# semihkacmaz/CoNFiLD

Hardware: AMD Instinct MI355X
Metric: generated fields/sec (256-step sample + CNF decode), Case4 latent, 1/2/4/8 GPU (higher is better)
Workload: dtype f32

## Files before the change

confild_amd/csrc/conv_x.hip:

```cpp
#include <algorithm>
#include <type_traits>

#include "unet_kernels.hpp"

namespace cfd {

typedef float f16v __attribute__((ext_vector_type(16)));
typedef float f2 __attribute__((ext_vector_type(2)));
typedef _Float16 h2 __attribute__((ext_vector_type(2)));
typedef unsigned u4 __attribute__((ext_vector_type(4)));

__device__ __forceinline__ int xswz(int row, int chunk) { return row * 64 + ((chunk ^ ((row >> 2) & 3)) << 4); }

__device__ __forceinline__ void split4_mix_x(const f4& x, uint2& hi, uint2& lo) {
    hi.x = __builtin_bit_cast(unsigned, __builtin_convertvector((f2){x[0], x[1]}, h2));
    hi.y = __builtin_bit_cast(unsigned, __builtin_convertvector((f2){x[2], x[3]}, h2));
    asm("v_fma_mixlo_f16 %0, %1, 1.0, -%2 op_sel_hi:[0,0,1]" : "=&v"(lo.x) : "v"(x[0]), "v"(hi.x));
    asm("v_fma_mixhi_f16 %0, %1, 1.0, -%2 op_sel:[0,0,1] op_sel_hi:[0,0,1]" : "+v"(lo.x) : "v"(x[1]), "v"(hi.x));
    asm("v_fma_mixlo_f16 %0, %1, 1.0, -%2 op_sel_hi:[0,0,1]" : "=&v"(lo.y) : "v"(x[2]), "v"(hi.y));
    asm("v_fma_mixhi_f16 %0, %1, 1.0, -%2 op_sel:[0,0,1] op_sel_hi:[0,0,1]" : "+v"(lo.y) : "v"(x[3]), "v"(hi.y));
}

__device__ __forceinline__ float phase_scale(const ConvArgs& a, int ph) {
    return ph == 0 ? a.ph_scale[0] : ph == 1 ? a.ph_scale[1] : ph == 2 ? a.ph_scale[2] : a.ph_scale[3];
}

template <int BM, int BN, int WGM, int WGN, int PF = 1, bool PH = false>
__global__ __launch_bounds__(64 * WGM * WGN, 1) void conv_x_kernel(ConvArgs a) {
    constexpr int NW = WGM * WGN, NT = 64 * NW;
    constexpr int WTM = BM / WGM, WTN = BN / WGN;
    constexpr int TM = WTM / 32, TN = WTN / 32;
    constexpr int RPP = NT / 8;
    constexpr int AIT = BM / RPP, BIT = BN / RPP;
    static_assert(TM >= 1 && TN >= 1 && AIT >= 1 && BIT >= 1, "tile");
    static_assert(BM % RPP == 0 && BN % RPP == 0, "staging");
    constexpr int ABYTES = BM * 64, BBYTES = BN * 64;
    constexpr int STAGE = 2 * ABYTES + 2 * BBYTES;
    __shared__ __attribute__((aligned(16))) char lds[2 * STAGE];

    CFD_STAMP(a.stamps, 2, a.seq, 0);
    const int tid = threadIdx.x, lane = tid & 63;
    const int wave = __builtin_amdgcn_readfirstlane(tid >> 6);
    const int wm = wave / WGN, wn = wave % WGN;

    int bx, by, bz;
    xcd_tile(a.xcd, bx, by, bz);
    const int ph = PH ? bx & 3 : 0, py = ph >> 1, px = ph & 1;
    if constexpr (PH) bx >>= 2;
    const int m0 = bx * BM, n0 = by * BN;
    const int HWo = a.Hout * a.Wout;
    const int HWm = PH ? a.Hin * a.Win : HWo, Wm = PH ? a.Win : a.Wout, Mm = PH ? a.M >> 2 : a.M;
    const int kq = tid & 7, rsub = tid >> 3;
    __shared__ int pixtab[(PH ? 4 : 9) * BM];

    const int srows = __builtin_amdgcn_readfirstlane(a.Hin * a.Win * (a.M / HWo));
// ... 176 lines not shown
    for (int i = 0; i < TM; ++i)
#pragma unroll
        for (int j = 0; j < TN; ++j) acc[i][j] *= PH ? phase_scale(a, ph) : a.acc_scale;
    const int n_base = n0 + wn * WTN + l32;
    const int m_base = m0 + wm * WTM + 4 * hsel;
    auto orow = [&](int mm, int& bb) __attribute__((always_inline)) {
        bb = mm / HWm;
        if constexpr (!PH) return mm;
        const int rem = mm - bb * HWm, y = rem / Wm, x = rem - y * Wm;
        return (bb * a.Hout + 2 * y + py) * a.Wout + 2 * x + px;
    };
    if (gridDim.z > 1) {
        float* part = a.part + (int64_t)bz * a.M * a.Cout;
#pragma unroll
        for (int i = 0; i < TM; ++i)
#pragma unroll
            for (int e = 0; e < 16; ++e) {
                const int mm = m_base + 32 * i + 8 * (e >> 2) + (e & 3);
                if (mm >= Mm) continue;
                int bb;
                const int m = orow(mm, bb);
#pragma unroll
                for (int j = 0; j < TN; ++j) {
                    const int n = n_base + 32 * j;
                    if (n < a.Cout) part[(int64_t)m * a.Cout + n] = acc[i][j][e];
                }
            }
#ifdef CFD_STAMPS
        __builtin_amdgcn_s_waitcnt(0);
#endif
        CFD_STAMP(a.stamps, 2, a.seq, 4);
        return;
    }
#pragma unroll
    for (int i = 0; i < TM; ++i)
#pragma unroll
        for (int e = 0; e < 16; ++e) {
            const int mm = m_base + 32 * i + 8 * (e >> 2) + (e & 3);
            if (mm >= Mm) continue;
            int bb;
            const int m = orow(mm, bb);
#pragma unroll
            for (int j = 0; j < TN; ++j) {
                const int n = n_base + 32 * j;
                if (n >= a.Cout) continue;
                float v = a.bias ? acc[i][j][e] + a.bias[n] : acc[i][j][e];
                if (a.emb) v = v + a.emb[(int64_t)bb * a.emb_stride + n];
                if (a.res) v = a.res[(int64_t)m * a.Cout + n] + v;
                a.out[(int64_t)m * a.Cout + n] = v;
            }
        }
}

template <int BM, int TW, bool BF = false, bool SB = false, int BN = 128, bool PH = false>
__global__ __launch_bounds__(BM * (BN / 64), 1) void conv_h_kernel(ConvArgs a) {
    static_assert(!SB || BF, "a bf16 source needs the bf16 kernel");
    static_assert(!PH || !BF, "the phase form is split-f16 only");
    constexpr unsigned SES = SB ? 2u : 4u;
    constexpr int WGN = BN / 64, WGM = BM / 64, NTG = 64 * WGM * WGN;
    static_assert(BN == 64 || BN == 128, "K1h: 64 or 128 output channels per workgroup");
    constexpr int PL = BF ? 1 : 2;
    constexpr int HW2 = TW < 32 ? (TW + 2 + 3) / 4 * 4 : TW + 2;
    constexpr int TR = BM / TW, NPX = (TR + 2) * HW2;
    auto hswz = [](int px, int hr, int chunk) __attribute__((always_inline)) {
        if constexpr (TW == 16) return px * 64 + ((chunk ^ (((px >> 2) + 3 * hr) & 3)) << 4);
        else return xswz(px, chunk);
    };
    constexpr int HPLANE = NPX * 64;
    constexpr int HIT = (NPX * 8 + NTG - 1) / NTG;
    constexpr int NTAP = PH ? 4 : 9;
    constexpr int TG = BF ? 3 : 1, SPR = NTAP / TG;
    constexpr int BPLANE = BN * 64, BSTAGE = PL * BPLANE * TG;
    constexpr int BIT = BN * 4 / NTG;
    constexpr int GBYTES = PL * HPLANE + 2 * BSTAGE;
    static_assert(BM % TW == 0 && BIT >= 1, "tile");
    __shared__ __attribute__((aligned(16))) char lds[GBYTES];

    CFD_STAMP(a.stamps, 3, a.seq, 0);
    const int tid = threadIdx.x, lane = tid & 63;
    const int wave = __builtin_amdgcn_readfirstlane(tid >> 6);
    const int wm = wave / WGN, wn = wave % WGN;
    const int gt = tid;
    char* const halo = lds;
    char* const ring = halo + PL * HPLANE;
    int bx, by, bz;
    xcd_tile(a.xcd, bx, by, bz);
    const int ph = PH ? bx & 3 : 0, py = ph >> 1, px = ph & 1;
    if constexpr (PH) bx >>= 2;
    const int n0 = by * BN;
    const int W = PH ? a.Win : a.Wout, Hh = PH ? a.Hin : a.Hout, HWo = Hh * W;
    const int tps = HWo / BM, tpr = W / TW;
    const int bimg = bx / tps, tl = bx - bimg * tps;
    const int y0 = (tl / tpr) * TR, x0 = (tl - (tl / tpr) * tpr) * TW;
    const int64_t mrow0 = PH ? ((int64_t)bimg * a.Hout + 2 * y0 + py) * a.Wout + 2 * x0 + px
                             : (int64_t)bimg * HWo + (int64_t)y0 * W + x0;
    CFD_DASSERT(mrow0 + (int64_t)(PH ? 2 : 1) * ((int64_t)(TR - 1) * a.Wout + TW - 1) < a.M && HWo % BM == 0 &&
                W % TW == 0);

    const int srows = __builtin_amdgcn_readfirstlane(a.Hin * a.Win * (a.M / (a.Hout * a.Wout)));
    const __amdgpu_buffer_rsrc_t rs1 = __builtin_amdgcn_make_buffer_rsrc((void*)a.src1, 0, srows * a.C1 * SES, 0x00020000);
    const __amdgpu_buffer_rsrc_t rs2 = __builtin_amdgcn_make_buffer_rsrc(
        (void*)(a.src2 ? (const void*)a.src2 : (const void*)a.src1), 0, a.src2 ? srows * a.C2 * SES : 0, 0x00020000);
    const int wbytes = a.Cout * NTAP * a.Ctot * 2;
    const char* const wh0 = PH ? (const char*)a.wph + (int64_t)ph * wbytes : (const char*)a.wbf;
    const char* const wl0 = PH ? (const char*)a.wpl + (int64_t)ph * wbytes : (const char*)a.wlo;
    const __amdgpu_buffer_rsrc_t rwh = __builtin_amdgcn_make_buffer_rsrc((void*)wh0, 0, wbytes, 0x00020000);
    const __amdgpu_buffer_rsrc_t rwl = __builtin_amdgcn_make_buffer_rsrc((void*)wl0, 0, wbytes, 0x00020000);

// ... 267 lines not shown
                const int64_t m = pix_of(p_base + 32 * i + 8 * (e >> 2) + (e & 3));
#pragma unroll
                for (int j = 0; j < 2; ++j) {
                    const int n = n_base + 32 * j;
                    if (n < a.Cout) part[(int64_t)m * a.Cout + n] = acc[i][j][e];
                }
            }
#ifdef CFD_STAMPS
        __builtin_amdgcn_s_waitcnt(0);
#endif
        CFD_STAMP(a.stamps, 3, a.seq, 4);
        return;
    }
#pragma unroll
    for (int i = 0; i < 2; ++i)
#pragma unroll
        for (int e = 0; e < 16; ++e) {
            const int64_t m = pix_of(p_base + 32 * i + 8 * (e >> 2) + (e & 3));
#pragma unroll
            for (int j = 0; j < 2; ++j) {
                const int n = n_base + 32 * j;
                if (n >= a.Cout) continue;
                float v = a.bias ? acc[i][j][e] + a.bias[n] : acc[i][j][e];
                if (a.emb) v = v + a.emb[(int64_t)bimg * a.emb_stride + n];
                if (a.res) v = a.res[(int64_t)m * a.Cout + n] + v;
                a.out[(int64_t)m * a.Cout + n] = v;
            }
        }
#ifdef CFD_STAMPS
    __builtin_amdgcn_s_waitcnt(0);
#endif
    CFD_STAMP(a.stamps, 3, a.seq, 4);
}

int conv_h_tw(const ConvArgs& a) {
    const bool geo = !a.tmode && a.ks == 3 && a.stride == 1 && a.pad == 1 && a.C1 % 32 == 0 && a.C2 % 32 == 0 &&
                     (a.up ? a.Hout == 2 * a.Hin && a.Wout == 2 * a.Win : a.Hout == a.Hin && a.Wout == a.Win) &&
                     a.M % (a.Hout * a.Wout) == 0;
    if (!geo) return 0;
    for (int tw = 64; tw >= 16; tw >>= 1)
        if (a.Wout % tw == 0 && a.Hout % (256 / tw) == 0) return tw;
    return 0;
}

int conv_hp_tw(const ConvArgs& a) {
    const bool geo = !a.tmode && a.up && a.ks == 3 && a.stride == 1 && a.pad == 1 && a.C1 % 32 == 0 &&
                     a.C2 % 32 == 0 && a.Hout == 2 * a.Hin && a.Wout == 2 * a.Win && a.M % (a.Hout * a.Wout) == 0;
    if (!geo) return 0;
    for (int tw = 64; tw >= 16; tw >>= 1)
        if (a.Win % tw == 0 && a.Hin % (256 / tw) == 0) return tw;
    return 0;
}

int launch_conv_x(const ConvArgs& a, int variant, int splits, hipStream_t st) {
    CFD_REQUIRE(a.wbf && !a.tmode, CFD_ESTATE, "conv_x: split-f16 or bf16 forward only");
    CFD_REQUIRE(a.Ctot % 32 == 0 && a.C1 % 4 == 0 && a.C2 % 4 == 0, CFD_ESHAPE, "conv_x needs channels % 32 == 0");
    CFD_REQUIRE(splits == 1 || a.part, CFD_ESTATE, "split-K needs a partial buffer");
    {
        const int64_t srows = (int64_t)a.Hin * a.Win * (a.M / (a.Hout * a.Wout));
        CFD_REQUIRE(srows < (1 << 24) && srows * std::max(a.C1, a.C2) * 4 < (1ll << 31) &&
                        (int64_t)a.Cout * a.K * 2 < (1ll << 31) && a.ks * a.ks <= 9,
                    CFD_ESHAPE, "conv_x: operands beyond 2 GiB");
    }
    auto grid = [&](int bm, int bn) __attribute__((always_inline)) {
        return dim3((unsigned)ceil_div(a.M, bm), (unsigned)ceil_div(a.Cout, bn), splits);
    };
    if (variant == 22) {
        const int tw = conv_h_tw(a);
        CFD_REQUIRE(tw > 0 && !a.wlo, CFD_ESHAPE, "conv_h bf16: 3x3 stride-1 with a 16/32/64-divisible width");
        const dim3 g = grid(256, 128);
        if (a.src_bf16) {
            if (tw == 64) hipLaunchKernelGGL((conv_h_kernel<256, 64, true, true>), g, dim3(512), 0, st, a);
            else if (tw == 32) hipLaunchKernelGGL((conv_h_kernel<256, 32, true, true>), g, dim3(512), 0, st, a);
            else hipLaunchKernelGGL((conv_h_kernel<256, 16, true, true>), g, dim3(512), 0, st, a);
        } else {
            if (tw == 64) hipLaunchKernelGGL((conv_h_kernel<256, 64, true>), g, dim3(512), 0, st, a);
            else if (tw == 32) hipLaunchKernelGGL((conv_h_kernel<256, 32, true>), g, dim3(512), 0, st, a);
            else hipLaunchKernelGGL((conv_h_kernel<256, 16, true>), g, dim3(512), 0, st, a);
        }
        check_launch("conv_h_kernel");
        return splits;
    }
    CFD_REQUIRE(!a.src_bf16, CFD_ESTATE, "internal: a bf16 convolution source needs the K1hb kernel");
    if (variant == 20) {
        const int tw = conv_h_tw(a);
        CFD_REQUIRE(tw > 0, CFD_ESHAPE, "conv_h: 3x3 stride-1 with a 16/32/64-divisible width");
        static const int smalln = smalln_below();
        const dim3 g = grid(256, 128);
        if ((int64_t)g.x * g.y * g.z < smalln && a.Cout % 64 == 0) {
            const dim3 g64 = grid(256, 64);
            if (tw == 64) hipLaunchKernelGGL((conv_h_kernel<256, 64, false, false, 64>), g64, dim3(256), 0, st, a);
            else if (tw == 32) hipLaunchKernelGGL((conv_h_kernel<256, 32, false, false, 64>), g64, dim3(256), 0, st, a);
            else hipLaunchKernelGGL((conv_h_kernel<256, 16, false, false, 64>), g64, dim3(256), 0, st, a);
            check_launch("conv_h_kernel");
            return splits;
        }
        if (tw == 64) hipLaunchKernelGGL((conv_h_kernel<256, 64>), g, dim3(512), 0, st, a);
        else if (tw == 32) hipLaunchKernelGGL((conv_h_kernel<256, 32>), g, dim3(512), 0, st, a);
        else hipLaunchKernelGGL((conv_h_kernel<256, 16>), g, dim3(512), 0, st, a);
        check_launch("conv_h_kernel");
        return splits;
    }
    CFD_REQUIRE(a.wlo, CFD_ESTATE, "internal: K1x runs split-f16 operands only");
    if (variant >= 24 && variant <= 26) {
        CFD_REQUIRE(a.wph && a.wpl && a.up && a.ks == 3 && a.stride == 1 && a.pad == 1 && a.Hout == 2 * a.Hin &&
                        a.Wout == 2 * a.Win,
                    CFD_ESTATE, "internal: the phase form needs an Upsample convolution and its phase packs");
        if (variant == 24) {
            const int tw = conv_hp_tw(a);
            CFD_REQUIRE(tw > 0, CFD_ESHAPE, "conv_h phase form: a 16/32/64-divisible low-resolution width");
            const dim3 g = grid(256, 128);
            if (tw == 64) hipLaunchKernelGGL((conv_h_kernel<256, 64, false, false, 128, true>), g, dim3(512), 0, st, a);
            else if (tw == 32) hipLaunchKernelGGL((conv_h_kernel<256, 32, false, false, 128, true>), g, dim3(512), 0, st, a);
            else hipLaunchKernelGGL((conv_h_kernel<256, 16, false, false, 128, true>), g, dim3(512), 0, st, a);
            check_launch("conv_h_kernel (phase)");
            return splits;
        }
        const int bm = variant == 26 ? 256 : 128;
        const dim3 g(4u * (unsigned)ceil_div(a.M / 4, bm), (unsigned)ceil_div(a.Cout, 128), splits);
        if (variant == 26) hipLaunchKernelGGL((conv_x_kernel<256, 128, 4, 2, 1, true>), g, dim3(512), 0, st, a);
        else hipLaunchKernelGGL((conv_x_kernel<128, 128, 2, 2, 1, true>), g, dim3(256), 0, st, a);
        check_launch("conv_x_kernel (phase)");
        return splits;
    }
    switch (variant) {
        case 1: hipLaunchKernelGGL((conv_x_kernel<128, 128, 2, 2>), grid(128, 128), dim3(256), 0, st, a); break;
        case 2: hipLaunchKernelGGL((conv_x_kernel<256, 128, 4, 2>), grid(256, 128), dim3(512), 0, st, a); break;
        default: CFD_REQUIRE(false, CFD_EARG, "conv_x variant");
    }
    check_launch("conv_x_kernel");
    return splits;
}

}
```

confild_amd/csrc/unet.hip:

```cpp
#include <algorithm>
#include <cstring>
#include <cmath>
#include <functional>
#include <map>
#include <string>
#include <vector>

#include "sampler.hpp"
#include "unet_kernels.hpp"
#include "unet_train.hpp"

namespace cfd {

enum class Pack { Raw, Conv3, Conv1, EmbW, EmbB };

struct UParam {
    std::string key;
    std::vector<int64_t> shape;
    Pack pack = Pack::Raw;
    size_t offset = 0;
    size_t count = 0;
    int emb_row = 0;
    bool set = false;
    int tpack = 0;
// ... 807 lines not shown
        a.Win = X.W;
        a.Hout = Hout;
        a.Wout = Wout;
        a.ks = ks;
        a.stride = stride;
        a.pad = pad;
        a.up = up;
        a.bpart = wbpart;
        a.bpart_cap = (int64_t)bcap;
        a.Gb = GP(pre + ".bias");
        if (!cfd::launch_conv_wgrad(a, GP(pre + ".weight"), st)) {
            cfd::launch_colsum(dy, a.P, cout, 1, cpart, crow, st);
            cfd::launch_rows_accum(crow, 1, cout, GP(pre + ".bias"), st);
        }
        return a.amax_y;
    };
    if (pg) CFD_HIP(hipMemsetAsync(demb, 0, sizeof(float) * B * h->tdim, st));
    if (split_w) CFD_HIP(hipMemsetAsync(wamax, 0, sizeof(unsigned) * kRangeSlots, st));

    auto gfree = [&](const float* b1, const float* b2 = nullptr, const float* b3 = nullptr) -> float* {
        for (auto p : gpool)
            if (p != b1 && p != b2 && p != b3) return p;
        throw cfd::Error{CFD_ESTATE, "internal: gradient pool exhausted"};
    };
    auto dconv = [&](const float* dy, int cin, int Hin, int Win, const std::string& key, int cout, int Hout, int Wout,
                     int ks, int stride, int pad, int tmode, float* out) {
        {
            auto it = h->index.find(key);
            CFD_REQUIRE(it != h->index.end(), CFD_EKEY, "internal: missing conv " + key);
            const int tp = h->params[it->second].tpack;
            CFD_REQUIRE((tp == 3 && tmode == 0) || (tp == 1 && tmode == 1) || (tp == 2 && tmode == 0) ||
                            (tp == 1 && ks == 1),
                        CFD_ESTATE, "internal: input-gradient pack kind / addressing mismatch at " + key);
        }
        cfd::ConvArgs a{};
        a.src1 = dy;
        a.C1 = cin;
        a.Ctot = cin;
        a.w = PT(h, key);
        PTS(h, key, &a);
        a.out = out;
        a.part = splitk;
        a.Hin = Hin;
        a.Win = Win;
        a.Hout = Hout;
        a.Wout = Wout;
        a.stride = stride;
        a.ks = ks;
        a.pad = pad;
        a.tmode = tmode;
        a.Cout = cout;
        a.M = B * Hout * Wout;
        a.K = ks * ks * cin;
        cfd::launch_conv(a, plan_checked(h, a, kSplitCap), st);
    };
    auto gnb = [&](const Act& in, const float* ss, const float* stats, const std::string& pre, int silu,
                   const float* dz, const float* addsrc, float* out1, float* out2, bool with_param = false,
                   unsigned* amax_out = nullptr) {
        cfd::GnbArgs g{};
        g.x1 = in.a;
        g.x2 = in.b;
        g.dz = dz;
        g.ss = ss;
        g.stats = stats;
        g.gamma = P(h, pre + ".weight");
        g.addsrc = addsrc;
        g.out1 = out1;
        g.out2 = out2;
        g.part = gnpart;
        g.fin = gnfin;
        g.C1 = in.Ca;
        g.C2 = in.Cb;
        g.Ctot = in.C();
        g.HW = in.H * in.W;
        g.silu = silu;
        g.plan_b = plan_batch(h);
        if (with_param && pg) g.ppart = gpp;
        g.amax_out = amax_out;
        const int nch = cfd::launch_gn_bwd(g, B, st);
        if (g.ppart)
            cfd::launch_gn_param_accum(gpp, B * nch, g.Ctot, GP(pre + ".weight"), GP(pre + ".bias"), st);
    };

    Act dcur;
    unsigned* dmax = nullptr;
    for (size_t si = h->steps.size(); si-- > 0;) {
        const auto& s = h->steps[si];
        const Rec& r = recs[si];
        const Act& in = r.in;
        switch (s.kind) {
            case cfd::Step::Out: {
                float* G = gpool[0];
                cfd::ConvArgs a{};
                a.src1 = d_eps;
                a.C1 = c.out_channels;
                a.Ctot = c.out_channels;
                a.w = PT(h, "out.2.weight");
                a.out = G;
                a.Hin = a.Hout = in.H;
                a.Win = a.Wout = in.W;
                a.Cout = in.Ca;
                a.M = B * in.H * in.W;
                a.tmode = 1;
                cfd::launch_conv_in(a, st);
                float* dh = gpool[1];
                unsigned* hm = slot();
                gnb(in, r.ss1, r.st1, "out.0", 1, G, nullptr, dh, nullptr, true, hm);
// ... 696 lines not shown
            for (int64_t i = 0; i < Cin; ++i)
                for (int tap = 0; tap < 9; ++tap) pk[(o * 9 + tap) * Cin + i] = w_host[(o * Cin + i) * 9 + tap];
        float amax = 0.f;
        for (float v : pk) amax = std::max(amax, std::fabs(v));
        int ex = 0;
        if (amax > 0.f) std::frexp(amax, &ex);
        const float s = std::ldexp(1.0f, -ex);
        std::vector<_Float16> hi(n), lo(n), phi, plo;
        for (size_t e = 0; e < n; ++e) {
            const float v = pk[e] * s;
            hi[e] = (_Float16)v;
            lo[e] = (_Float16)(v - (float)hi[e]);
        }
        cfd::ConvArgs a{};
        cfd::phase_pack_host(w_host, Cout, Cin, phi, plo, a.ph_scale);
        struct Bufs {
            void* p[7] = {};
            ~Bufs() { for (void* q : p) (void)hipFree(q); }
        } d;
        const size_t bytes[6] = {n * 4, n * 2, n * 2, phi.size() * 2, plo.size() * 2, (size_t)Cout * 4};
        const void* srcs[6] = {pk.data(), hi.data(), lo.data(), phi.data(), plo.data(), bias_host};
        for (int k = 0; k < 6; ++k) {
            CFD_HIP(hipMalloc(&d.p[k], bytes[k]));
            CFD_HIP(hipMemcpy(d.p[k], srcs[k], bytes[k], hipMemcpyHostToDevice));
        }
        a.src1 = x;
        a.C1 = a.Ctot = Cin;
        a.w = (const float*)d.p[0];
        a.wbf = d.p[1];
        a.wlo = d.p[2];
        a.wph = d.p[3];
        a.wpl = d.p[4];
        a.acc_scale = std::ldexp(1.0f, ex);
        a.bias = (const float*)d.p[5];
        a.out = out;
        a.Hin = H;
        a.Win = W;
        a.Hout = 2 * H;
        a.Wout = 2 * W;
        a.stride = 1;
        a.ks = 3;
        a.pad = 1;
        a.up = 1;
        a.Cout = Cout;
        a.M = B * a.Hout * a.Wout;
        a.K = 9 * Cin;
        a.plan_b = plan_b > 0 ? plan_b : 8;
        const cfd::ConvPlan plan = cfd::plan_conv(a, kSplitPer8);
        if (plan.splits > 1) {
            CFD_HIP(hipMalloc(&d.p[6], sizeof(float) * plan.splits * (size_t)a.M * Cout));
            a.part = (float*)d.p[6];
        }
        if (kx) *kx = plan.kx;
        cfd::launch_conv(a, plan, st);
        CFD_HIP(hipStreamSynchronize(st));
    });
}

extern "C" int cfd_unet_set_compute(cfd_unet* h, int compute) {
    return cfd::guard([&] {
        CFD_REQUIRE(h, CFD_EARG, "null handle");
        CFD_REQUIRE(compute == CFD_COMPUTE_F32 || compute == CFD_COMPUTE_BF16 || compute == CFD_COMPUTE_SPLIT_F16,
                    CFD_EARG, "unknown compute mode");
        if (h->compute != compute) ++h->version;
        h->compute = compute;
    });
}

extern "C" int cfd_unet_set_plan_batch(cfd_unet* h, int nominal_batch) {
    return cfd::guard([&] {
        CFD_REQUIRE(h, CFD_EARG, "null handle");
        CFD_REQUIRE(nominal_batch >= 0 && nominal_batch <= 64, CFD_EARG, "plan batch must be 0 (default) .. 64");
        if (h->plan_b != nominal_batch) {
            ++h->version;
            h->ws_cache.clear();
        }
        h->plan_b = nominal_batch;
    });
}

extern "C" int cfd_unet_set_time_freqs(cfd_unet* h, const float* host, int n) {
    return cfd::guard([&] {
        CFD_REQUIRE(h && host && n == h->cfg.model_channels / 2, CFD_EARG, "freqs must have model_channels/2 entries");
        cfd::DeviceGuard dg(h->device);
        CFD_HIP(hipMemcpy(h->freqs, host, sizeof(float) * n, hipMemcpyHostToDevice));
    });
}

extern "C" int cfd_unet_ready(const cfd_unet* h) {
    return cfd::guard([&] {
        CFD_REQUIRE(h, CFD_EARG, "null handle");
        for (const auto& p : h->params) CFD_REQUIRE(p.set, CFD_ESTATE, "U-Net parameter not set: " + p.key);
    });
}

namespace cfd {
size_t unet_ws_bytes(const cfd_unet* h, int B) {
    auto it = h->ws_cache.find(B);
    if (it != h->ws_cache.end()) return it->second;
    Workspace ws{nullptr, 0, true};
    run(h, nullptr, nullptr, nullptr, B, ws, nullptr);
    h->ws_cache[B] = ws.off + 256;
    return ws.off + 256;
}
void unet_check_ready(const cfd_unet* h) {
    for (const auto& p : h->params) CFD_REQUIRE(p.set, CFD_ESTATE, "U-Net parameter not set: " + p.key);
// ... 186 lines not shown
```

confild_amd/csrc/unet_kernels.hip:

```cpp
#include <algorithm>
#include <cstdlib>

#include "unet_kernels.hpp"

namespace cfd {

__global__ __launch_bounds__(256) void gn_partial_kernel(GnArgs a) {
    const int chunk = blockIdx.x;
    const int64_t b = blockIdx.y;
    const int Ctot = a.Ctot, cq = Ctot / 4, cpg = Ctot / 32;
    const int HW = a.HW;
    const int p0 = (int)((int64_t)HW * chunk / a.nchunks), p1 = (int)((int64_t)HW * (chunk + 1) / a.nchunks);
    const int rows = 256 / cq;
    const int q = threadIdx.x % cq, r0 = threadIdx.x / cq;
    __shared__ double red[2][1024];
    if (r0 < rows) {
        double s[4] = {0, 0, 0, 0}, s2[4] = {0, 0, 0, 0};
        const int c0 = 4 * q;
        for (int p = p0 + r0; p < p1; p += rows) {
            const int64_t pix = b * HW + p;
            const f4 v = c0 < a.C1 ? *(const f4*)(a.src1 + pix * a.C1 + c0)
                                   : *(const f4*)(a.src2 + pix * a.C2 + (c0 - a.C1));
#pragma unroll
            for (int j = 0; j < 4; ++j) {
// ... 1765 lines not shown
    const int64_t srows = (int64_t)a.Hin * a.Win * (a.M / (a.Hout * a.Wout));
    return force_k1s || !(srows < (1 << 24) && a.M < (1 << 24) && srows * std::max(a.C1, a.C2) * 4 < (1ll << 31));
}

static bool conv_p_falls_back(const ConvArgs& a) {
    return !conv_p_applies(a) || (int64_t)a.Cout * a.K * 2 >= (1ll << 31);
}

bool conv_runs_k1hb(const ConvArgs& a, const ConvPlan& p) { return p.kx == 22 && !conv_x_falls_back(a); }

bool conv_kv_pack_ok(const ConvArgs& a, const ConvPlan& p, int T) {
    static const int ldsepi = env_int("CFD_CONV_LDSEPI", 1);
    return ldsepi && (p.kx < 0 || p.kx >= 40) && p.splits == 1 && a.wbf && !a.tmode && a.ks == 1 && a.bias &&
           !a.emb && !a.res && a.Cout % 8 == 0 && a.emb_stride % 4 == 0 && T % 32 == 0 && a.M % T == 0;
}

int launch_conv(const ConvArgs& a, const ConvPlan& p0, hipStream_t st, bool defer) {
    ConvPlan p = p0;
    if (p.kx >= 0 && (conv_x_falls_back(a) || (p.kx >= 40 && conv_p_falls_back(a)))) {
        p.kx = -1;
        p.bm = p.bn = 128;
        p.nw = 8;
    }
    CFD_REQUIRE(!a.src_bf16 || p.kx == 22, CFD_ESTATE, "internal: a bf16 convolution source needs the K1hb kernel");
    static const int pf = env_int("CFD_CONV_PF", 2);
    if (p.kx < 0) p.pf = pf >= 1 && pf <= 3 ? pf : 1;
    CFD_REQUIRE(a.Ctot % 32 == 0 && a.C1 % 4 == 0 && a.C2 % 4 == 0, CFD_ESHAPE, "conv_gemm needs channels % 32 == 0");
    CFD_REQUIRE(a.K == a.ks * a.ks * a.Ctot, CFD_ESHAPE, "conv K mismatch");
    CFD_REQUIRE(p.splits == 1 || (a.part && a.Cout % 4 == 0), CFD_ESTATE, "split-K needs a partial buffer");
    CFD_REQUIRE(!a.tmode || ((a.stride == 1 || a.stride == 2) && !a.up), CFD_ESHAPE, "transposed conv: stride 1|2");
    const dim3 grid((unsigned)ceil_div(a.M, p.bm), (unsigned)ceil_div(a.Cout, p.bn), p.splits);
    CFD_REQUIRE(!(a.tmode && a.wbf && !a.wlo), CFD_ESTATE, "bf16 input-gradient convolutions are not built");
    static const int xcd = env_int("CFD_CONV_XCD", 4);
    static const int ldsepi = env_int("CFD_CONV_LDSEPI", 1);
    ConvArgs b = a;
    b.stamps = g_stamps;
    b.seq = g_seq++;
    b.ldsepi = ldsepi && a.Cout % 4 == 0 && a.emb_stride % 4 == 0;
    const int xo = xcd == 4 ? (a.wbf && !a.wlo ? 1 : 3) : xcd;
    b.xcd = xo == 3 ? ((int64_t)a.Hout * a.Wout <= 256 ? 2 : 1) : xo < 0 || xo > 2 ? 1 : xo;
    {
        const int64_t srows = (int64_t)a.Hin * a.Win * (a.M / (a.Hout * a.Wout));
        const int64_t wes = (a.wbf || a.wlo) ? 2 : 4;
        b.bufaddr = a.ks * a.ks <= 9 && srows < (1 << 24) && a.M < (1 << 24) &&
                    srows * std::max(a.C1, a.C2) * 4 < (1ll << 31) && (int64_t)a.Cout * a.K * wes < (1ll << 31);
    }
    const ConvArgs& a_ = b;
    if (p.kx >= 40) {
        CFD_REQUIRE(p.splits == 1, CFD_ESTATE, "internal: K1p does not split over K");
        launch_conv_p(a_, p.kx, st);
        return 1;
    }
    if (p.kx >= 0) {
        launch_conv_x(a_, p.kx, p.splits, st);
        if (p.splits > 1 && !defer) launch_splitk_reduce(a, p.splits, st);
        return p.splits;
    }
    if (a.tmode && a.wlo)
        launch_conv_tiles<true, 2>(a_, p, grid, st);
    else if (a.tmode)
        launch_conv_tiles<true, 0>(a_, p, grid, st);
    else if (a.wbf && a.wlo)
        launch_conv_tiles<false, 2>(a_, p, grid, st);
    else if (a.wbf)
        launch_conv_tiles<false, 1>(a_, p, grid, st);
    else
        launch_conv_tiles<false, 0>(a_, p, grid, st);
    check_launch("conv_gemm_kernel");
    if (p.splits > 1 && !defer) launch_splitk_reduce(a, p.splits, st);
    return p.splits;
}

void launch_conv_in(const ConvArgs& a, hipStream_t st) {
    if (a.Cout % 4 == 0 && a.C1 <= 4 && (size_t)9 * a.C1 * a.Cout * 4 <= 64 * 1024) {
        const int64_t n = (int64_t)a.M * (a.Cout / 4);
        hipLaunchKernelGGL(conv_in_vec_kernel, dim3((unsigned)std::min<int64_t>(2048, ceil_div(n, 256))), dim3(256),
                           sizeof(float) * 9 * a.C1 * a.Cout, st, a);
        check_launch("conv_in_vec_kernel");
        return;
    }
    const int64_t n = (int64_t)a.M * a.Cout;
    hipLaunchKernelGGL(conv_in_kernel, dim3((unsigned)ceil_div(n, 256)), dim3(256), 0, st, a);
    check_launch("conv_in_kernel");
}

void launch_conv_out(const ConvArgs& a, hipStream_t st) {
    CFD_REQUIRE(a.Cout <= 4, CFD_ESHAPE, "out_channels must be <= 4");
    const int LP = a.Ctot / 4;
    if (a.Ctot % 4 == 0 && a.C1 == a.Ctot && LP >= 1 && LP <= 64 && (LP & (LP - 1)) == 0 &&
        (size_t)a.Cout * a.K * 4 <= 64 * 1024) {
        const int64_t waves = ceil_div(a.M, 64 / LP);
        hipLaunchKernelGGL(conv_out_vec_kernel, dim3((unsigned)std::min<int64_t>(8192, ceil_div(waves, 4))), dim3(256),
                           sizeof(float) * a.Cout * a.K, st, a, LP);
        check_launch("conv_out_vec_kernel");
        return;
    }
    hipLaunchKernelGGL(conv_out_kernel, dim3((unsigned)ceil_div(a.M, 4)), dim3(256), 0, st, a);
    check_launch("conv_out_kernel");
}

void launch_attention(const AttnArgs& a, int CH, int heads, int B, hipStream_t st) {
    const dim3 grid((unsigned)ceil_div(a.T, 64), heads, B);
    switch (CH) {
        case 16: hipLaunchKernelGGL(attention_kernel<16>, grid, dim3(256), 0, st, a); break;
        case 32: hipLaunchKernelGGL(attention_kernel<32>, grid, dim3(256), 0, st, a); break;
        case 64: hipLaunchKernelGGL(attention_kernel<64>, grid, dim3(256), 0, st, a); break;
        case 128: hipLaunchKernelGGL(attention_kernel<128>, grid, dim3(256), 0, st, a); break;
// ... 107 lines not shown
```

confild_amd/csrc/unet_kernels.hpp:

```cpp
#pragma once
#include <algorithm>
#include <cmath>
#include <vector>

#include "common.hpp"

namespace cfd {

struct GnArgs {
    const float* src1;
    const float* src2;
    const float* gamma;
    const float* beta;
    double* part;
    float* ss;
    float* out;
    float* stats;
    int C1, C2, Ctot, HW;
    float eps;
    int silu;
    int nchunks;
    int B;
    const float* kpart;
    const float* kbias;
// ... 88 lines not shown

void stamps_set(unsigned long long* buf);
unsigned long long* stamps_buf();

struct AttnArgs {
    const float* qkv;
    float* out;
    int T, C;
    float scale;
    float* lse;
    int xcdmap;
    int kc;
    float* part;
};

struct GnbArgs {
    const float* x1;
    const float* x2;
    const float* dz;
    const float* ss;
    const float* stats;
    const float* gamma;
    const float* addsrc;
    float* out1;
    float* out2;
    int acc1, acc2;
    double* part;
    float* fin;
    float* ppart;
    unsigned* amax_out;
    int C1, C2, Ctot, HW, silu, nchunks, B;
    int plan_b;
};

struct AttnBwdArgs {
    const float* qkv;
    const float* o;
    const float* dout;
    const float* lse;
    float* dd;
    float* dqkv;
    int T, C;
    float scale;
    h8v* packs;
    float* amax;
    int heads, xcdmap;
};

struct ConvPlan {
    int bm = 128, bn = 128, splits = 1;
    int nw = 4;
    int kx = -1;
    int pf = 1;
};

constexpr int kGnMaxChunks = 512;
int gn_chunks(int HW);
constexpr int kGn2BigHW = 16384, kGn2BigChunks = 256;
static_assert(kGn2BigChunks <= kGnMaxChunks, "gn2 partials live in the kGnMaxChunks slab");
int gn2_chunks(int HW, int plan_b);
inline int gn2_threads(int nchunks) { return nchunks > 64 ? 1024 : 256; }
void launch_gn(const GnArgs& a, int B, hipStream_t st);
bool gn_takes_splitk(const GnArgs& a, int B);
bool gn2_applies(const GnArgs& a);
ConvPlan plan_conv(const ConvArgs& a, size_t part_cap_floats);
int launch_conv(const ConvArgs& a, const ConvPlan& p, hipStream_t st, bool defer = false);
void launch_splitk_reduce(const ConvArgs& a, int splits, hipStream_t st);
__device__ __forceinline__ void xcd_tile(int order, int& bx, int& by, int& bz) {
    bx = blockIdx.x;
    by = blockIdx.y;
    bz = blockIdx.z;
    if (!order) return;
    const unsigned gx = gridDim.x, gy = gridDim.y, gz = gridDim.z;
    const unsigned T = gx * gy * gz, L = blockIdx.x + gx * (blockIdx.y + gy * blockIdx.z);
    const unsigned q = T >> 3, r = T & 7, x = L & 7, sl = L >> 3;
    const unsigned Lp = x < r ? x * (q + 1) + sl : r * (q + 1) + (x - r) * q + sl;
    if (order == 2) {
        bx = Lp % gx;
        bz = (Lp / gx) % gz;
        by = Lp / (gx * gz);
    } else {
        bz = Lp % gz;
        by = (Lp / gz) % gy;
        bx = Lp / (gz * gy);
    }
}
int launch_conv_x(const ConvArgs& a, int variant, int splits, hipStream_t st);
int conv_h_tw(const ConvArgs& a);
int conv_hp_tw(const ConvArgs& a);
bool conv_p_applies(const ConvArgs& a);
void conv_p_tile(int variant, int& bm, int& bn, int& nw);
void launch_conv_p(const ConvArgs& a, int variant, hipStream_t st);
int smalln_below();
bool conv_runs_k1hb(const ConvArgs& a, const ConvPlan& p);
void launch_conv_in(const ConvArgs& a, hipStream_t st);
void launch_conv_out(const ConvArgs& a, hipStream_t st);
void launch_attention(const AttnArgs& a, int CH, int heads, int B, hipStream_t st);
size_t attention_split_floats(int T, int C);
int attention_kv_chunks(int T, int heads, int plan_b);
size_t attention_part_floats(int T, int C, int CH, int plan_b);
void launch_attention_split(const AttnArgs& a, int CH, int heads, int B, int plan_b, float* kvws, hipStream_t st,
                            bool packed);
int64_t attention_split_voff(int T, int CH, int heads, int B);
bool conv_kv_pack_ok(const ConvArgs& a, const ConvPlan& p, int T);
int launch_gn_bwd(const GnbArgs& a, int B, hipStream_t st);
void launch_attention_bwd(const AttnBwdArgs& a, int CH, int heads, int B, hipStream_t st);
size_t attention_bwd_split_floats(int T, int C);
bool attention_bwd_split_ok(int T, int CH);
void launch_attention_bwd_split(const AttnBwdArgs& a, int CH, int heads, int B, float* ws, hipStream_t st);
void launch_add(float* y, const float* x, int64_t n, hipStream_t st);
void launch_temb(const int64_t* t, const float* freqs, float* out, int dim, int B, hipStream_t st);
void launch_linear(const float* x, const float* W, const float* bias, float* y, int B, int K, int N, int act,
                   hipStream_t st);


__device__ __forceinline__ float kln2(float scale) { return scale * 1.44269504088896340736f; }
__device__ __forceinline__ void split8_f16(const float (&v)[8], h8v& hi, h8v& lo) {
#pragma clang fp contract(off)
#pragma unroll
    for (int t = 0; t < 8; ++t) {
        hi[t] = (_Float16)v[t];
        lo[t] = (_Float16)(v[t] - (float)hi[t]);
    }
}
constexpr int vmcnt_wait(int n) { return (n & 15) | (7 << 4) | (15 << 8) | (((n >> 4) & 3) << 14); }
}
```

Measured before the change: 4.067.

## Add 16x16x32 MFMA body for split-f16 halo convolution and make it default

Adds a new body for the halo-tiled 3x3 convolution kernel that uses 16x16x32 f16 MFMA fragments instead of the 32x32 form. It comes with a new LDS swizzle/offset layout header, double-buffered per-tap weight staging, and an optional LDS-staged epilogue. The forward path, including the phase form, now picks the 16-wide shape by default, while the adjoint (backward) path keeps the 32 shape. The aim is better LDS access and scheduling for the split-f16 three-MFMA scheme, at the cost of a more complex kernel and new variant ids.

```diff
diff --git a/confild_amd/csrc/conv_x.hip b/confild_amd/csrc/conv_x.hip
--- a/confild_amd/csrc/conv_x.hip
+++ b/confild_amd/csrc/conv_x.hip
@@ -1,6 +1,7 @@
 #include <algorithm>
 #include <type_traits>
 
+#include "k1h_lds.hpp"
 #include "unet_kernels.hpp"
 
 namespace cfd {
@@ -283,8 +284,321 @@
         }
 }
 
-template <int BM, int TW, bool BF = false, bool SB = false, int BN = 128, bool PH = false>
+template <int V>
+using IC = std::integral_constant<int, V>;
+
+struct Tile3 {
+    int x, y, z;
+};
+__device__ __forceinline__ Tile3 xcd_tile_v(int order) {
+    if (!order) return Tile3{(int)blockIdx.x, (int)blockIdx.y, (int)blockIdx.z};
+    const unsigned gx = gridDim.x, gy = gridDim.y, gz = gridDim.z;
+    const unsigned T = gx * gy * gz, L = blockIdx.x + gx * (blockIdx.y + gy * blockIdx.z);
+    const unsigned q = T >> 3, r = T & 7, x = L & 7, sl = L >> 3;
+    const unsigned Lp = x < r ? x * (q + 1) + sl : r * (q + 1) + (x - r) * q + sl;
+    const bool o2 = order == 2;
+    const unsigned d1 = o2 ? gx : gz, d2 = o2 ? gz : gy;
+    const unsigned lo = Lp % d1, rest = Lp / d1, mid = rest % d2, hi = rest / d2;
+    return o2 ? Tile3{(int)lo, (int)hi, (int)mid} : Tile3{(int)hi, (int)mid, (int)lo};
+}
+
+template <int BM, int TW, int BN, bool PH>
+__device__ __forceinline__ void conv_h16_body(const ConvArgs& a) {
+    constexpr int WGN = BN / 64, WGM = BM / 64, NTG = 64 * WGM * WGN;
+    static_assert(BN == 64 || BN == 128, "K1h: 64 or 128 output channels per workgroup");
+    static_assert(TW == 16 || TW == 32 || TW == 64, "K1h: a 16-pixel fragment block lies in one tile row");
+    constexpr int HWD = TW + 2;
+    constexpr int TR = BM / TW, NPX = k1h_npx(BM, TW), NPXD = k1h_npx_staged(BM, TW);
+    constexpr int HPLANE = NPX * 64;
+    constexpr int HIT = (NPXD * 8 + NTG - 1) / NTG;
+    constexpr int NTAP = PH ? 4 : 9, TXN = PH ? 2 : 3;
+    constexpr int BPLANE = BN * 64, BSTAGE = 2 * BPLANE;
+    constexpr int BIT = BN * 4 / NTG;
+    constexpr int GBYTES = 2 * HPLANE + 2 * BSTAGE;
+    static_assert(BM % TW == 0 && BIT == 1 && BM % 64 == 0, "tile");
+    static_assert(k1h_a_imm(TW, 3, 2) + HPLANE + 3 * 64 + 64 < 65536, "fragment offsets are instruction offsets");
+    __shared__ __attribute__((aligned(16))) char lds[GBYTES];
+
+    CFD_STAMP(a.stamps, 3, a.seq, 0);
+    const int tid = threadIdx.x, lane = tid & 63;
+    const int wave = __builtin_amdgcn_readfirstlane(tid >> 6);
+    const int wm = wave / WGN, wn = wave % WGN;
+    const int gt = tid;
+    char* const halo = lds;
+    char* const ring = halo + 2 * HPLANE;
+    const Tile3 wg = xcd_tile_v(a.xcd);
+    int bx = wg.x;
+    const int by = wg.y, bz = wg.z;
+    const int ph = PH ? bx & 3 : 0, py = ph >> 1, px = ph & 1;
+    if constexpr (PH) bx >>= 2;
+    const int n0 = by * BN;
+    const int W = PH ? a.Win : a.Wout, Hh = PH ? a.Hin : a.Hout, HWo = Hh * W;
+    const int tps = HWo / BM, tpr = W / TW;
+    const int bimg = bx / tps, tl = bx - bimg * tps;
+    const int y0 = (tl / tpr) * TR, x0 = (tl - (tl / tpr) * tpr) * TW;
+    const int64_t mrow0 = PH ? ((int64_t)bimg * a.Hout + 2 * y0 + py) * a.Wout + 2 * x0 + px
+                             : (int64_t)bimg * HWo + (int64_t)y0 * W + x0;
+    CFD_DASSERT(mrow0 + (int64_t)(PH ? 2 : 1) * ((int64_t)(TR - 1) * a.Wout + TW - 1) < a.M && HWo % BM == 0 &&
+                W % TW == 0);
+
+    const int srows = __builtin_amdgcn_readfirstlane(a.Hin * a.Win * (a.M / (a.Hout * a.Wout)));
+    const __amdgpu_buffer_rsrc_t rs1 = __builtin_amdgcn_make_buffer_rsrc((void*)a.src1, 0, srows * a.C1 * 4, 0x00020000);
+    const __amdgpu_buffer_rsrc_t rs2 = __builtin_amdgcn_make_buffer_rsrc(
+        (void*)(a.src2 ? (const void*)a.src2 : (const void*)a.src1), 0, a.src2 ? srows * a.C2 * 4 : 0, 0x00020000);
+    const int wbytes = a.Cout * NTAP * a.Ctot * 2;
+    const char* const wh0 = PH ? (const char*)a.wph + (int64_t)ph * wbytes : (const char*)a.wbf;
+    const char* const wl0 = PH ? (const char*)a.wpl + (int64_t)ph * wbytes : (const char*)a.wlo;
+    const __amdgpu_buffer_rsrc_t rwh = __builtin_amdgcn_make_buffer_rsrc((void*)wh0, 0, wbytes, 0x00020000);
+    const __amdgpu_buffer_rsrc_t rwl = __builtin_amdgcn_make_buffer_rsrc((void*)wl0, 0, wbytes, 0x00020000);
+
+    const int kq = gt & 7;
+    int hpix[HIT], hst[HIT];
+#pragma unroll
+    for (int it = 0; it < HIT; ++it) {
+        const int hp = (gt + it * NTG) >> 3;
+        int pix = -1;
+        hst[it] = 0;
+        if (hp < NPXD) {
+            const int hr = hp / HWD, hc = hp - hr * HWD;
+            const int iy = y0 - 1 + hr + py, ix = x0 - 1 + hc + px;
+            if ((!PH || (hc < TW + 1 && hr < TR + 1)) && iy >= 0 && iy < Hh && ix >= 0 && ix < W)
+                pix = a.up && !PH ? (bimg * a.Hin + (iy >> 1)) * a.Win + (ix >> 1) : (bimg * a.Hin + iy) * a.Win + ix;
+            hst[it] = k1h_stage_off(TW, hp, kq);
+            CFD_DASSERT(hst[it] >= 0 && hst[it] + 8 <= HPLANE);
+        }
+        CFD_DASSERT(pix < srows);
+        hpix[it] = pix;
+    }
+    const int bq = gt & 3;
+    const int nrow = n0 + (gt >> 2);
+    const unsigned bvoff = nrow < a.Cout ? (unsigned)((nrow * NTAP * a.Ctot + 8 * bq) * 2) : 0x80000000u;
+    const int wst = k1h_wstage_off(gt >> 2, bq);
+
+    const int nch = a.Ctot / 32;
+    const int per = (nch + gridDim.z - 1) / gridDim.z;
+    const int c0 = bz * per, cend = min(nch, c0 + per);
+    const int nrounds = max(cend - c0, 0);
+
+    f4 rh[HIT];
+    u4 wx_h, wx_l, wy_h, wy_l;
+    auto load_halo = [&](int c) __attribute__((always_inline)) {
+        const int cb = 32 * c;
+        const bool second = cb >= a.C1;
+        const unsigned csrc = 4u * (unsigned)(second ? a.C2 + 0 : a.C1 + 0);
+        const unsigned cofs = c < nch ? 4u * ((second ? cb - a.C1 : cb) + 4 * kq) : 0x80000000u;
+        if (second) {
+#pragma unroll
+            for (int it = 0; it < HIT; ++it) {
+                const unsigned off = hpix[it] >= 0 ? __umul24((unsigned)hpix[it], csrc) + cofs : 0x80000000u;
+                rh[it] = __builtin_bit_cast(f4, __builtin_amdgcn_raw_buffer_load_b128(rs2, off, 0, 0));
+            }
+        } else {
+#pragma unroll
+            for (int it = 0; it < HIT; ++it) {
+                const unsigned off = hpix[it] >= 0 ? __umul24((unsigned)hpix[it], csrc) + cofs : 0x80000000u;
+                rh[it] = __builtin_bit_cast(f4, __builtin_amdgcn_raw_buffer_load_b128(rs1, off, 0, 0));
+            }
+        }
+    };
+    auto store_halo = [&]() __attribute__((always_inline)) {
+#pragma unroll
+        for (int it = 0; it < HIT; ++it) {
+            if (gt + it * NTG < NPXD * 8) {
+                uint2 hv, lv;
+                split4_mix_x(rh[it], hv, lv);
+                *(uint2*)(halo + hst[it]) = hv;
+                *(uint2*)(halo + HPLANE + hst[it]) = lv;
+            }
+        }
+    };
+    auto load_w = [&](int c, int t, u4& rbh, u4& rbl) __attribute__((always_inline)) {
+        const int soff = (t * a.Ctot + 32 * min(c, cend - 1)) * 2;
+        rbh = __builtin_bit_cast(u4, __builtin_amdgcn_raw_buffer_load_b128(rwh, bvoff, soff, 0));
+        rbl = __builtin_bit_cast(u4, __builtin_amdgcn_raw_buffer_load_b128(rwl, bvoff, soff, 0));
+    };
+    auto store_w = [&](int stage, const u4& rbh, const u4& rbl) __attribute__((always_inline)) {
+        char* base = ring + stage * BSTAGE + wst;
+        *(u4*)base = rbh;
+        *(u4*)(base + BPLANE) = rbl;
+    };
+
+    f4 acc[4][4];
+#pragma unroll
+    for (int i = 0; i < 4; ++i)
+#pragma unroll
+        for (int j = 0; j < 4; ++j) acc[i][j] = f4{0.f, 0.f, 0.f, 0.f};
+
+    const int li = lane & 15, g = lane >> 4;
+    const char* abase[TXN];
+#pragma unroll
+    for (int tx = 0; tx < TXN; ++tx) abase[tx] = halo + k1h_a_base(TW, wm, li, g, tx);
+    const char* const bbase = ring + k1h_b_base(wn, li, g);
+    CFD_DASSERT(k1h_a_base(TW, wm, li, g, TXN - 1) + k1h_a_imm(TW, 3, PH ? 1 : 2) + 16 <= HPLANE);
+
+    auto step = [&](int r, auto tc, auto qc, u4& ldh, u4& ldl, const u4& sth, const u4& stl)
+        __attribute__((always_inline)) {
+        constexpr int T = decltype(tc)::value, Q = decltype(qc)::value;
+        constexpr int ty = PH ? T >> 1 : T / 3, tx = PH ? T & 1 : T - 3 * ty;
+        const int c = c0 + r;
+        load_w(T + 2 < NTAP ? c : c + 1, (T + 2) % NTAP, ldh, ldl);
+        if constexpr (T == 0) load_halo(r + 1 < nrounds ? c + 1 : nch);
+        const char* const ap = abase[tx];
+        const char* const bp = bbase + Q * BSTAGE;
+        h8v fbh[4], fbl[4];
+#pragma unroll
+        for (int j = 0; j < 4; ++j) {
+            fbh[j] = *(const h8v*)(bp + k1h_b_imm(j));
+            fbl[j] = *(const h8v*)(bp + BPLANE + k1h_b_imm(j));
+        }
+#pragma unroll
+        for (int i = 0; i < 4; ++i) {
+            const h8v fah = *(const h8v*)(ap + k1h_a_imm(TW, i, ty));
+            const h8v fal = *(const h8v*)(ap + HPLANE + k1h_a_imm(TW, i, ty));
+#pragma unroll
+            for (int j = 0; j < 4; ++j) acc[i][j] = __builtin_amdgcn_mfma_f32_16x16x32_f16(fal, fbh[j], acc[i][j], 0, 0, 0);
+#pragma unroll
+            for (int j = 0; j < 4; ++j) acc[i][j] = __builtin_amdgcn_mfma_f32_16x16x32_f16(fah, fbl[j], acc[i][j], 0, 0, 0);
+#pragma unroll
+            for (int j = 0; j < 4; ++j) acc[i][j] = __builtin_amdgcn_mfma_f32_16x16x32_f16(fah, fbh[j], acc[i][j], 0, 0, 0);
+        }
+        store_w(Q ^ 1, sth, stl);
+        __syncthreads();
+        if constexpr (T == NTAP - 1) {
+            store_halo();
+            __syncthreads();
+        }
+        __builtin_amdgcn_sched_barrier(0);
+    };
+    auto round = [&](int r, auto q0c) __attribute__((always_inline)) {
+        constexpr int Q0 = decltype(q0c)::value;
+        auto tap = [&](auto tc) __attribute__((always_inline)) {
+            constexpr int Q = (Q0 + decltype(tc)::value) & 1;
+            if constexpr (Q == 0) step(r, tc, IC<0>{}, wx_h, wx_l, wy_h, wy_l);
+            else step(r, tc, IC<1>{}, wy_h, wy_l, wx_h, wx_l);
+        };
+        tap(IC<0>{}), tap(IC<1>{}), tap(IC<2>{}), tap(IC<3>{});
+        if constexpr (!PH) tap(IC<4>{}), tap(IC<5>{}), tap(IC<6>{}), tap(IC<7>{}), tap(IC<8>{});
+    };
+
+    if (nrounds > 0) {
+        load_w(c0, 0, wx_h, wx_l);
+        load_w(c0, 1, wy_h, wy_l);
+        load_halo(c0);
+        store_w(0, wx_h, wx_l);
+        store_halo();
+        __syncthreads();
+        CFD_STAMP(a.stamps, 3, a.seq, 2);
+        if constexpr (NTAP & 1) {
+            int r = 0;
+            for (; r + 2 <= nrounds; r += 2) {
+                round(r, IC<0>{});
+                round(r + 1, IC<1>{});
+            }
+            if (r < nrounds) round(r, IC<0>{});
+        } else {
+            for (int r = 0; r < nrounds; ++r) round(r, IC<0>{});
+        }
+    }
+
+    CFD_STAMP(a.stamps, 3, a.seq, 3);
+    const float scl = PH ? phase_scale(a, ph) : a.acc_scale;
+#pragma unroll
+    for (int i = 0; i < 4; ++i)
+#pragma unroll
+        for (int j = 0; j < 4; ++j) acc[i][j] *= scl;
+    auto pix_of = [&](int p) __attribute__((always_inline)) {
+        if constexpr (PH) return mrow0 + (int64_t)(p / TW) * (2 * a.Wout) + 2 * (p % TW);
+        else return mrow0 + (int64_t)(p / TW) * W + (p % TW);
+    };
+    if (a.ldsepi) {
+        static_assert(64 * BN * 4 <= GBYTES, "epilogue stage fits the LDS");
+        float* stg = (float*)lds;
+        const bool split = gridDim.z > 1;
+        float* dstb = split ? a.part + (int64_t)bz * a.M * a.Cout : a.out;
+        constexpr int Q = BN / 4;
+        __syncthreads();
+        for (int r = 0; r < WGM; ++r) {
+            if (wm == r) {
+#pragma unroll
+                for (int i = 0; i < 4; ++i)
+#pragma unroll
+                    for (int j = 0; j < 4; ++j)
+#pragma unroll
+                        for (int e = 0; e < 4; ++e)
+                            stg[k1h_epi(BN, 16 * i + 4 * g + e, wn * 64 + 16 * j + li)] = acc[i][j][e];
+            }
+            __syncthreads();
+            for (int q = tid; q < 64 * Q; q += NTG) {
+                const int p = q / Q, c = (q - p * Q) * 4;
+                const int n = n0 + c;
+                if (n < a.Cout) {
+                    const int64_t m = pix_of(r * 64 + p);
+                    f4 v = *(const f4*)(stg + k1h_epi(BN, p, c));
+                    if (!split) {
+                        if (a.bias) v = v + *(const f4*)(a.bias + n);
+                        if (a.emb) v = v + *(const f4*)(a.emb + (int64_t)bimg * a.emb_stride + n);
+                        if (a.res) v = *(const f4*)(a.res + m * a.Cout + n) + v;
+                    }
+                    *(f4*)(dstb + m * a.Cout + n) = v;
+                }
+            }
+            __syncthreads();
+        }
+#ifdef CFD_STAMPS
+        __builtin_amdgcn_s_waitcnt(0);
+#endif
+        CFD_STAMP(a.stamps, 3, a.seq, 4);
+        return;
+    }
+    const int n_base = n0 + wn * 64 + li;
+    const int p_base = wm * 64 + 4 * g;
+    if (gridDim.z > 1) {
+        float* part = a.part + (int64_t)bz * a.M * a.Cout;
+#pragma unroll
+        for (int i = 0; i < 4; ++i)
+#pragma unroll
+            for (int e = 0; e < 4; ++e) {
+                const int64_t m = pix_of(p_base + 16 * i + e);
+#pragma unroll
+                for (int j = 0; j < 4; ++j) {
+                    const int n = n_base + 16 * j;
+                    if (n < a.Cout) part[m * a.Cout + n] = acc[i][j][e];
+                }
+            }
+#ifdef CFD_STAMPS
+        __builtin_amdgcn_s_waitcnt(0);
+#endif
+        CFD_STAMP(a.stamps, 3, a.seq, 4);
+        return;
+    }
+#pragma unroll
+    for (int i = 0; i < 4; ++i)
+#pragma unroll
+        for (int e = 0; e < 4; ++e) {
+            const int64_t m = pix_of(p_base + 16 * i + e);
+#pragma unroll
+            for (int j = 0; j < 4; ++j) {
+                const int n = n_base + 16 * j;
+                if (n >= a.Cout) continue;
+                float v = a.bias ? acc[i][j][e] + a.bias[n] : acc[i][j][e];
+                if (a.emb) v = v + a.emb[(int64_t)bimg * a.emb_stride + n];
+                if (a.res) v = a.res[m * a.Cout + n] + v;
+                a.out[m * a.Cout + n] = v;
+            }
+        }
+#ifdef CFD_STAMPS
+    __builtin_amdgcn_s_waitcnt(0);
+#endif
+    CFD_STAMP(a.stamps, 3, a.seq, 4);
+}
+
+template <int BM, int TW, bool BF = false, bool SB = false, int BN = 128, bool PH = false, int SHAPE = 32>
 __global__ __launch_bounds__(BM * (BN / 64), 1) void conv_h_kernel(ConvArgs a) {
+    static_assert(SHAPE == 32 || (SHAPE == 16 && !BF && !SB), "K1h: 16x16x32 is the split-f16 form's");
+    if constexpr (SHAPE == 16) {
+        conv_h16_body<BM, TW, BN, PH>(a);
+        return;
+    }
     static_assert(!SB || BF, "a bf16 source needs the bf16 kernel");
     static_assert(!PH || !BF, "the phase form is split-f16 only");
     constexpr unsigned SES = SB ? 2u : 4u;
@@ -658,7 +972,30 @@
     return 0;
 }
 
-int launch_conv_x(const ConvArgs& a, int variant, int splits, hipStream_t st) {
+int k1h_shape(int tw, int bn, bool phase, bool adjoint) {
+    (void)tw, (void)bn, (void)phase;
+#ifdef CFD_K1H_MFMA32
+    (void)adjoint;
+    return 32;
+#else
+    return adjoint ? 32 : 16;
+#endif
+}
+
+template <int BN, bool PH, int SHAPE>
+static void launch_h_(const ConvArgs& a, int tw, dim3 g, hipStream_t st) {
+    const dim3 blk(256 * (BN / 64));
+    if (tw == 64) hipLaunchKernelGGL((conv_h_kernel<256, 64, false, false, BN, PH, SHAPE>), g, blk, 0, st, a);
+    else if (tw == 32) hipLaunchKernelGGL((conv_h_kernel<256, 32, false, false, BN, PH, SHAPE>), g, blk, 0, st, a);
+    else hipLaunchKernelGGL((conv_h_kernel<256, 16, false, false, BN, PH, SHAPE>), g, blk, 0, st, a);
+}
+template <int BN, bool PH>
+static void launch_h(const ConvArgs& a, int tw, int shape, dim3 g, hipStream_t st) {
+    if (shape == 16) launch_h_<BN, PH, 16>(a, tw, g, st);
+    else launch_h_<BN, PH, 32>(a, tw, g, st);
+}
+
+int launch_conv_x(const ConvArgs& a, int variant, int splits, hipStream_t st, bool adjoint) {
     CFD_REQUIRE(a.wbf && !a.tmode, CFD_ESTATE, "conv_x: split-f16 or bf16 forward only");
     CFD_REQUIRE(a.Ctot % 32 == 0 && a.C1 % 4 == 0 && a.C2 % 4 == 0, CFD_ESHAPE, "conv_x needs channels % 32 == 0");
     CFD_REQUIRE(splits == 1 || a.part, CFD_ESTATE, "split-K needs a partial buffer");
@@ -688,37 +1025,32 @@
         return splits;
     }
     CFD_REQUIRE(!a.src_bf16, CFD_ESTATE, "internal: a bf16 convolution source needs the K1hb kernel");
-    if (variant == 20) {
+    if (variant == 20 || variant == 32 || variant == 33) {
         const int tw = conv_h_tw(a);
-        CFD_REQUIRE(tw > 0, CFD_ESHAPE, "conv_h: 3x3 stride-1 with a 16/32/64-divisible width");
+        CFD_REQUIRE(tw > 0 && a.wlo, CFD_ESHAPE, "conv_h: split-f16 3x3 stride-1 with a 16/32/64-divisible width");
         static const int smalln = smalln_below();
         const dim3 g = grid(256, 128);
-        if ((int64_t)g.x * g.y * g.z < smalln && a.Cout % 64 == 0) {
-            const dim3 g64 = grid(256, 64);
-            if (tw == 64) hipLaunchKernelGGL((conv_h_kernel<256, 64, false, false, 64>), g64, dim3(256), 0, st, a);
-            else if (tw == 32) hipLaunchKernelGGL((conv_h_kernel<256, 32, false, false, 64>), g64, dim3(256), 0, st, a);
-            else hipLaunchKernelGGL((conv_h_kernel<256, 16, false, false, 64>), g64, dim3(256), 0, st, a);
+        const bool n64 = (int64_t)g.x * g.y * g.z < smalln && a.Cout % 64 == 0;
+        const int shape = variant == 20 ? k1h_shape(tw, n64 ? 64 : 128, false, adjoint) : variant == 32 ? 32 : 16;
+        if (n64) {
+            launch_h<64, false>(a, tw, shape, grid(256, 64), st);
             check_launch("conv_h_kernel");
             return splits;
         }
-        if (tw == 64) hipLaunchKernelGGL((conv_h_kernel<256, 64>), g, dim3(512), 0, st, a);
-        else if (tw == 32) hipLaunchKernelGGL((conv_h_kernel<256, 32>), g, dim3(512), 0, st, a);
-        else hipLaunchKernelGGL((conv_h_kernel<256, 16>), g, dim3(512), 0, st, a);
+        launch_h<128, false>(a, tw, shape, g, st);
         check_launch("conv_h_kernel");
         return splits;
     }
     CFD_REQUIRE(a.wlo, CFD_ESTATE, "internal: K1x runs split-f16 operands only");
-    if (variant >= 24 && variant <= 26) {
+    if ((variant >= 24 && variant <= 26) || variant == 34 || variant == 35) {
         CFD_REQUIRE(a.wph && a.wpl && a.up && a.ks == 3 && a.stride == 1 && a.pad == 1 && a.Hout == 2 * a.Hin &&
                         a.Wout == 2 * a.Win,
                     CFD_ESTATE, "internal: the phase form needs an Upsample convolution and its phase packs");
-        if (variant == 24) {
+        if (variant == 24 || variant == 34 || variant == 35) {
             const int tw = conv_hp_tw(a);
             CFD_REQUIRE(tw > 0, CFD_ESHAPE, "conv_h phase form: a 16/32/64-divisible low-resolution width");
             const dim3 g = grid(256, 128);
-            if (tw == 64) hipLaunchKernelGGL((conv_h_kernel<256, 64, false, false, 128, true>), g, dim3(512), 0, st, a);
-            else if (tw == 32) hipLaunchKernelGGL((conv_h_kernel<256, 32, false, false, 128, true>), g, dim3(512), 0, st, a);
-            else hipLaunchKernelGGL((conv_h_kernel<256, 16, false, false, 128, true>), g, dim3(512), 0, st, a);
+            launch_h<128, true>(a, tw, variant == 24 ? k1h_shape(tw, 128, true, adjoint) : variant == 34 ? 32 : 16, g, st);
             check_launch("conv_h_kernel (phase)");
             return splits;
         }
diff --git a/confild_amd/csrc/k1h_lds.hpp b/confild_amd/csrc/k1h_lds.hpp
--- /dev/null
+++ b/confild_amd/csrc/k1h_lds.hpp
@@ -0,0 +1,24 @@
+#pragma once
+
+namespace cfd {
+
+constexpr int k1h_swz(int row, int chunk, bool swz = true) {
+    return row * 64 + ((chunk + (swz ? 2 * ((row >> 2) & 1) : 0)) & 3) * 16;
+}
+constexpr int k1h_hws(int tw) { return (tw + 2 + 7) / 8 * 8; }
+constexpr int k1h_npx(int bm, int tw) { return (bm / tw + 2) * k1h_hws(tw); }
+constexpr int k1h_npx_staged(int bm, int tw) { return (bm / tw + 2) * (tw + 2); }
+constexpr int k1h_stage_px(int tw, int hp) { return (hp / (tw + 2)) * k1h_hws(tw) + hp % (tw + 2); }
+constexpr int k1h_stage_off(int tw, int hp, int kq, bool swz = true) {
+    return k1h_swz(k1h_stage_px(tw, hp), kq >> 1, swz) + (kq & 1) * 8;
+}
+constexpr int k1h_a_base(int tw, int wm, int li, int g, int tx, bool swz = true) {
+    return k1h_swz((wm * 64 / tw) * k1h_hws(tw) + li + tx, g, swz);
+}
+constexpr int k1h_a_imm(int tw, int i, int ty) { return ((16 * i / tw + ty) * k1h_hws(tw) + 16 * i % tw) * 64; }
+constexpr int k1h_b_base(int wn, int li, int g, bool swz = true) { return k1h_swz(wn * 64 + li, g, swz); }
+constexpr int k1h_b_imm(int j) { return 16 * j * 64; }
+constexpr int k1h_wstage_off(int row, int bq, bool swz = true) { return k1h_swz(row, bq, swz); }
+constexpr int k1h_epi(int bn, int row, int col) { return row * bn + (col ^ (((row >> 2) & 3) << 4)); }
+
+}
diff --git a/confild_amd/csrc/unet.hip b/confild_amd/csrc/unet.hip
--- a/confild_amd/csrc/unet.hip
+++ b/confild_amd/csrc/unet.hip
@@ -883,7 +883,9 @@
         a.Cout = cout;
         a.M = B * Hout * Wout;
         a.K = ks * ks * cin;
-        cfd::launch_conv(a, plan_checked(h, a, kSplitCap), st);
+        cfd::ConvPlan plan = plan_checked(h, a, kSplitCap);
+        plan.adjoint = true;
+        cfd::launch_conv(a, plan, st);
     };
     auto gnb = [&](const Act& in, const float* ss, const float* stats, const std::string& pre, int silu,
                    const float* dz, const float* addsrc, float* out1, float* out2, bool with_param = false,
@@ -1686,6 +1688,11 @@
             a.part = (float*)d.p[6];
         }
         if (kx) *kx = plan.kx;
+        static const int conv_log = getenv("CFD_CONV_LOG") ? atoi(getenv("CFD_CONV_LOG")) : 0;
+        if (conv_log)
+            fprintf(stderr, "CONV upsample_conv %dx%d C=%d+%d->%d ks=%d s=%d up=%d M=%d kx=%d bm=%d bn=%d nw=%d splits=%d\n",
+                    a.Hin, a.Win, a.C1, a.C2, a.Cout, a.ks, a.stride, a.up, a.M, plan.kx, plan.bm, plan.bn, plan.nw,
+                    plan.splits);
         cfd::launch_conv(a, plan, st);
         CFD_HIP(hipStreamSynchronize(st));
     });
diff --git a/confild_amd/csrc/unet_kernels.hip b/confild_amd/csrc/unet_kernels.hip
--- a/confild_amd/csrc/unet_kernels.hip
+++ b/confild_amd/csrc/unet_kernels.hip
@@ -1841,7 +1841,7 @@
         return 1;
     }
     if (p.kx >= 0) {
-        launch_conv_x(a_, p.kx, p.splits, st);
+        launch_conv_x(a_, p.kx, p.splits, st, p.adjoint);
         if (p.splits > 1 && !defer) launch_splitk_reduce(a, p.splits, st);
         return p.splits;
     }
diff --git a/confild_amd/csrc/unet_kernels.hpp b/confild_amd/csrc/unet_kernels.hpp
--- a/confild_amd/csrc/unet_kernels.hpp
+++ b/confild_amd/csrc/unet_kernels.hpp
@@ -164,6 +164,7 @@
     int nw = 4;
     int kx = -1;
     int pf = 1;
+    bool adjoint = false;
 };
 
 constexpr int kGnMaxChunks = 512;
@@ -197,9 +198,10 @@
         bx = Lp / (gz * gy);
     }
 }
-int launch_conv_x(const ConvArgs& a, int variant, int splits, hipStream_t st);
+int launch_conv_x(const ConvArgs& a, int variant, int splits, hipStream_t st, bool adjoint = false);
 int conv_h_tw(const ConvArgs& a);
 int conv_hp_tw(const ConvArgs& a);
+int k1h_shape(int tw, int bn, bool phase, bool adjoint);
 bool conv_p_applies(const ConvArgs& a);
 void conv_p_tile(int variant, int& bm, int& bn, int& nw);
 void launch_conv_p(const ConvArgs& a, int variant, hipStream_t st);
```

New measurement: 4.148 (median of 6 runs). +2.0%, better.
